# facebookresearch/PartDistillation

Hardware: AMD Instinct MI355X
Metric: images/sec training step, R50 Mask2Former 1024² bs=2/GPU, 1/2/4/8 MI355X (higher is better)
Workload: dtype bf16

## Files before the change

include/pd_gemm.h:

```cpp
#ifndef PD_GEMM_H
#define PD_GEMM_H

#include <stdint.h>

#ifdef __cplusplus
extern "C" {
#endif

int pd_gemm_tn_f32(const float *A, const float *B, const float *bias, float *C, int M, int N, int K, int lda, int ldb,
                   int ldc, int relu, void *stream);

int pd_gemm_tn_f32x3(const float *A, const float *B, const float *bias, float *C, int M, int N, int K, int lda, int ldb,
                     int ldc, int relu, void *stream);

int pd_gemm_wgrad_f32(const float *dY, const float *X, float *dW, float *dB, int M, int N, int K, int ldy, int ldx,
                      int ldw, void *stream);

int pd_gemm_wgrad_acc_f32(const float *dY, const float *X, float *dW, float *dB, int M, int N, int K, int ldy, int ldx,
                          int ldw, void *stream);

int64_t pd_gemm_tn_f32x3_relu_bits_words(int M, int N);
int pd_split3_bf16(const float *W, int N, int K, int ldw, int transpose, void *planes, void *stream);
int pd_gemm_tn_f32x3_pre(const float *A, const void *Bplanes, const float *bias, float *C, uint32_t *bits, float *colsum, int M, int N, int K,
                         int lda, int ldc, int mode, void *stream);
int pd_gemm_tn_f32x3_relu_bits(const float *A, const float *B, const float *bias, float *C, uint32_t *bits, int M, int N, int K, int lda,
                               int ldb, int ldc, void *stream);
int pd_gemm_tn_f32x3_relumask(const float *A, const float *B, const uint32_t *bits, float *C, float *colsum, int M, int N, int K, int lda,
                              int ldb, int ldc, void *stream);

int pd_gemm_wgrad_acc_f32x3(const float *dY, const float *X, float *dW, float *dB, int M, int N, int K, int ldy, int ldx, int ldw,
                            void *stream);
int64_t pd_gemm_wgrad_f32x3_ws_floats(int N, int K);
int pd_gemm_wgrad_acc_f32x3_ws(const float *dY, const float *X, float *dW, float *dB, float *workspace, int64_t workspace_floats, int M, int N,
                               int K, int ldy, int ldx, int ldw, void *stream);

typedef struct PdGemmWgradDesc {
  const float *dY, *X;
  float *dW, *dB;
  int M, N, K, ldy, ldx, ldw;
  const float *y_amax, *x_amax;
} PdGemmWgradDesc;
int64_t pd_gemm_wgrad_f32x3_grouped_table_bytes(int max_count);
int64_t pd_gemm_wgrad_f32x3_grouped_ws_floats(const PdGemmWgradDesc *descs, int count);
int pd_gemm_wgrad_f32x3_grouped(const PdGemmWgradDesc *descs, int count, void *table_host_pinned, void *table_device, float *workspace,
                                int64_t workspace_floats, void *stream);

int pd_conv3x3_wgrad_nhwc_f32x3(const float *dY, const float *X, float *dWk, float *dB, float *workspace, int64_t workspace_floats, int B, int H,
                                int W, int Ci, int Co, void *stream);

int pd_conv3x3_nhwc_f32x3(const float *X, const float *Wk, const float *bias, float *Y, int B, int H, int W, int Ci, int Co,
                          void *stream);

int64_t pd_gemm_wgrad_f16x2_ws_floats(int N, int K);
int pd_gemm_wgrad_f16x2_takes_wide_tiles(int N, int K);
int64_t pd_gemm_wgrad_f16x2_grouped_ws_floats(const PdGemmWgradDesc *descs, int count);
int pd_gemm_wgrad_acc_f16x2_ws(const float *dY, const float *X, float *dW, float *dB, const float *y_amax, const float *x_amax,
                               float *workspace, int64_t workspace_floats, int M, int N, int K, int ldy, int ldx, int ldw, void *stream);
int pd_gemm_wgrad_f16x2_grouped(const PdGemmWgradDesc *descs, int count, void *table_host_pinned, void *table_device, float *workspace,
                                int64_t workspace_floats, void *stream);
int pd_conv3x3_wgrad_nhwc_f16x2(const float *dY, const float *X, float *dWk, float *dB, const float *y_amax, const float *x_amax,
                                float *workspace, int64_t workspace_floats, int B, int H, int W, int Ci, int Co, void *stream);
int pd_gemm_tn_f16x2_which(int M, int N, int K, int mode, int has_bits, int has_amax);

int pd_conv3x3_nhwc_f16x2(const float *X, const float *Wk, const float *bias, float *Y, const float *x_amax, const float *w_amax, float *y_amax,
                          int B, int H, int W, int Ci, int Co, void *stream);
int64_t pd_gemm_tn_f16x2_bits_words(int M, int N);
int pd_gemm_tn_f16x2(const float *A, const float *B, const float *bias, float *C, uint32_t *bits, float *colsum, const float *a_amax,
                     const float *b_amax, float *c_amax, int M, int N, int K, int lda, int ldb, int ldc, int mode, void *stream);
int pd_row_amax_f32(const float *X, int rows, int cols, int ld, float *out, void *stream);
int pd_gemm_tn_f16x2_bf16out(const float *A, const float *B, const float *bias, void *C_bf16, const float *a_amax, const float *b_amax, int M, int N,
                             int K, int lda, int ldb, int ldc, void *stream);
int pd_cast_bf16_f32_amax(const void *X_bf16, int rows, int cols, float *Y, float *row_amax, void *stream);

#ifdef __cplusplus
}
#endif
#endif
```

partdistillation_amd/csrc/common.hip:

```cpp
#include <hip/hip_runtime.h>
#include <stdarg.h>
#include <stdio.h>
#include <string.h>

#include "pd_common.h"
#include "pd_msda.h"

namespace {
thread_local char g_err[512] = {0};
}

int pd_set_error(int code, const char *fmt, ...)
{
  va_list ap;
  va_start(ap, fmt);
  vsnprintf(g_err, sizeof(g_err), fmt, ap);
  va_end(ap);
  return code;
}

int pd_check_launch(const char *what)
{
  hipError_t e = hipGetLastError();
  if (e == hipSuccess) return PD_OK;
  return pd_set_error(PD_ERR_LAUNCH, "%s: %s", what, hipGetErrorString(e));
}

extern "C" const char *pd_last_error(void) { return g_err; }
extern "C" int pd_abi_version(void) { return 39; }

extern int g_pd_dbg_atomic_scope;
extern int g_pd_dbg_force_generic;
extern int g_pd_dbg_ablate;
extern int g_pd_dbg_x3_narrow;
extern int g_pd_dbg_f16x2;
extern int g_pd_dbg_wgrad_wide;
extern "C" void pd_dbg_set_wgrad_xcd(int v);
extern "C" void pd_dbg_set_wgrad_fast(int v);
extern int g_pd_dbg_bwd_variant;
extern int g_pd_dbg_msda_gate_pct;
extern int g_pd_dbg_wgrad_wgs;
extern int g_pd_dbg_bwd_threads;
extern int g_pd_dbg_attn_scalar;
extern int g_pd_dbg_wattn;
extern int g_pd_dbg_x3;
extern int g_pd_dbg_kmeans;
extern int g_pd_dbg_conv_group_rows;
extern int g_pd_dbg_conv_xcd_major;
extern int g_pd_dbg_sgemm_deep;
extern int g_ig_bn, g_ig_nst, g_ig_splits, g_ig_patch, g_ig_pcls;
extern int g_mx_bn, g_mx_nst;
extern int g_swin_ln_abl;
extern int g_ln_bwd_cap;
extern int g_crit_abl;
extern int g_attn_bwd_kc;
extern int g_wg_nst, g_wg_splits, g_wg_mode;
extern "C" int pd_debug_set(const char *key, int value)
{
  if (!key) return PD_ERR_INVALID_ARG;
  if (!strcmp(key, "msda_bwd_atomic_scope")) { g_pd_dbg_atomic_scope = value; return PD_OK; }
  if (!strcmp(key, "msda_ablate")) { g_pd_dbg_ablate = value; return PD_OK; }
  if (!strcmp(key, "msda_bwd_variant")) { g_pd_dbg_bwd_variant = value; return PD_OK; }
  if (!strcmp(key, "msda_gate_pct")) { g_pd_dbg_msda_gate_pct = value; return PD_OK; }
  if (!strcmp(key, "attn_scalar")) { g_pd_dbg_attn_scalar = value; return PD_OK; }
  if (!strcmp(key, "msda_bwd_threads")) { g_pd_dbg_bwd_threads = value; return PD_OK; }
  if (!strcmp(key, "wgrad_wgs")) { g_pd_dbg_wgrad_wgs = value; return PD_OK; }
  if (!strcmp(key, "kmeans_ablate")) { g_pd_dbg_kmeans = value; return PD_OK; }
  if (!strcmp(key, "wg_nst")) { g_wg_nst = value; return PD_OK; }
  if (!strcmp(key, "wg_splits")) { g_wg_splits = value; return PD_OK; }
  if (!strcmp(key, "wg_mode")) { g_wg_mode = value; return PD_OK; }
  if (!strcmp(key, "ig_bn")) { g_ig_bn = value; return PD_OK; }
  if (!strcmp(key, "ig_patch")) { g_ig_patch = value; return PD_OK; }
  if (!strcmp(key, "ig_pcls")) { g_ig_pcls = value; return PD_OK; }
  if (!strcmp(key, "ig_nst")) { g_ig_nst = value; return PD_OK; }
  if (!strcmp(key, "mx_bn")) { g_mx_bn = value; return PD_OK; }
  if (!strcmp(key, "attn_bwd_kc")) { g_attn_bwd_kc = value; return PD_OK; }
  if (!strcmp(key, "crit_abl")) { g_crit_abl = value; return PD_OK; }
  if (!strcmp(key, "ln_bwd_cap")) { g_ln_bwd_cap = value; return PD_OK; }
  if (!strcmp(key, "swin_ln_abl")) { g_swin_ln_abl = value; return PD_OK; }
  if (!strcmp(key, "mx_nst")) { g_mx_nst = value; return PD_OK; }
  if (!strcmp(key, "ig_splits")) { g_ig_splits = value; return PD_OK; }
  if (!strcmp(key, "sgemm_deep")) { g_pd_dbg_sgemm_deep = value; return PD_OK; }
  if (!strcmp(key, "conv_group_rows")) { g_pd_dbg_conv_group_rows = value; return PD_OK; }
  if (!strcmp(key, "conv_xcd_major")) { g_pd_dbg_conv_xcd_major = value; return PD_OK; }
  if (!strcmp(key, "x3_ablate")) { g_pd_dbg_x3 = value; return PD_OK; }
  if (!strcmp(key, "f16x2_tile")) { g_pd_dbg_f16x2 = value; return PD_OK; }
  if (!strcmp(key, "wgrad_wide")) { g_pd_dbg_wgrad_wide = value; return PD_OK; }
  if (!strcmp(key, "wgrad_xcd")) { pd_dbg_set_wgrad_xcd(value); return PD_OK; }
  if (!strcmp(key, "wgrad_fast")) { pd_dbg_set_wgrad_fast(value); return PD_OK; }
  if (!strcmp(key, "x3_narrow")) { g_pd_dbg_x3_narrow = value; return PD_OK; }
  if (!strcmp(key, "wattn_ablate")) { g_pd_dbg_wattn = value; return PD_OK; }
  if (!strcmp(key, "msda_force_generic")) { g_pd_dbg_force_generic = value; return PD_OK; }
  return pd_set_error(PD_ERR_INVALID_ARG, "pd_debug_set: unknown key %s", key);
}
```

partdistillation_amd/csrc/gemm_f16x2.hip:

```cpp
#include <hip/hip_runtime.h>
#include <stdint.h>
#include <stdlib.h>
#include <type_traits>

#include "f16x2.h"
#include "pd_common.h"
#include "xcd.h"
#include "pd_gemm.h"
#include "pd_msda.h"

#ifndef PD_ABL
#define PD_ABL 0
#endif

namespace {
using namespace pdh2;
__device__ __forceinline__ int xcd_chunk(int bid, int nb) { return pd_xcd_chunk(bid, nb); }
__device__ __forceinline__ unsigned short f2bf_rne(float f)
{
  unsigned u = __float_as_uint(f);
  if ((u & 0x7fffffffu) > 0x7f800000u) return (unsigned short)((u >> 16) | 0x40u);
  u += 0x7fffu + ((u >> 16) & 1u);
  return (unsigned short)(u >> 16);
}
// ... 1023 lines not shown
      static bool battr = false;
      if (!battr) {
        (void)hipFuncSetAttribute((const void *)(gemm_kpc_f16x2<true, 0, true>), hipFuncAttributeMaxDynamicSharedMemorySize, (int)KP_LDS);
        (void)hipFuncSetAttribute((const void *)(gemm_kpc_f16x2<false, 0, true>), hipFuncAttributeMaxDynamicSharedMemorySize, (int)KP_LDS);
        (void)hipFuncSetAttribute((const void *)(gemm_kpc_f16x2<true, 16, true>), hipFuncAttributeMaxDynamicSharedMemorySize, (int)KP_LDS);
        battr = true;
      }
      const float *bpl = reinterpret_cast<const float *>(planes);
      if (dbg == 234) hipLaunchKernelGGL((gemm_kpc_f16x2<true, 16, true>), dim3((unsigned)G), dim3(768), KP_LDS, st, A, bpl, bias, C, M, K, lda, ldb, ldc, np, a_amax, b_amax, 0, 0);
      else if (a_amax) hipLaunchKernelGGL((gemm_kpc_f16x2<true, 0, true>), dim3((unsigned)G), dim3(768), KP_LDS, st, A, bpl, bias, C, M, K, lda, ldb, ldc, np, a_amax, b_amax, 0, 0);
      else hipLaunchKernelGGL((gemm_kpc_f16x2<false, 0, true>), dim3((unsigned)G), dim3(768), KP_LDS, st, A, bpl, bias, C, M, K, lda, ldb, ldc, np, a_amax, b_amax, 0, 0);
      return pd_check_launch("pd_gemm_tn_f16x2 (producer / consumer wavefronts, weight planes)");
    }
#endif
    if (a_amax) hipLaunchKernelGGL(gemm_kpc_f16x2<true>, dim3((unsigned)G), dim3(768), KP_LDS, st, A, B, bias, C, M, K, lda, ldb, ldc, np, a_amax, b_amax, 0, 0);
    else hipLaunchKernelGGL(gemm_kpc_f16x2<false>, dim3((unsigned)G), dim3(768), KP_LDS, st, A, B, bias, C, M, K, lda, ldb, ldc, np, a_amax, b_amax, 0, 0);
    return pd_check_launch("pd_gemm_tn_f16x2 (producer / consumer wavefronts)");
  }
  const bool need_wide = bits != nullptr;
  if (need_wide && ((N % 256) || M < 1024)) return pd_set_error(PD_ERR_INVALID_ARG, "pd_gemm_tn_f16x2: sign bits need N %% 256 == 0 and M >= 1024");
  const bool wide_ok = (N % 256) == 0 && M >= 1024;
  const bool by_shape = dbg == 0 || dbg == 61 || dbg == 70 || dbg == 80 || dbg == 62;
  static const bool wide_deepk = []() { const char *e = getenv("PD_H2_WIDE_DEEPK"); return e && e[0] == '1'; }();
  const bool wide = need_wide || dbg == 3 || dbg == 13 || (by_shape && wide_ok && (int64_t)((M + 255) / 256) * (N / 256) >= 128 && (N >= 1024 || (K >= 512 && wide_deepk)));
  static const bool fast_env = []() { const char *e = getenv("PD_H2_FAST"); return !e || e[0] != '0'; }();
#define GO(TM, TN, WN, NRS, FAST) return launch_f16x2<TM, TN, WN, 16, false, NRS, FAST>(A, B, bias, C, M, N, K, lda, ldb, ldc, mode, bits, colsum, a_amax, b_amax, c_amax, st, flags)
  if (wide) {
    if (!wide_ok) return pd_set_error(PD_ERR_INVALID_ARG, "pd_gemm_tn_f16x2: 256 x 256 tiles need N %% 256 == 0 and M >= 1024");
    if (dbg == 3) GO(256, 256, 128, 1, 0);
    if (dbg == 13 || dbg == 70) GO(256, 256, 128, 2, 0);
    if (!fast_env) GO(256, 256, 128, 2, 0);
    GO(256, 256, 128, 2, 1);
  }
  if (dbg == 4 || dbg == 70) GO(128, 128, 64, 1, 0);
  if (dbg == 14 || !fast_env) GO(128, 128, 64, 2, 0);
  GO(128, 128, 64, 2, 1);
#undef GO
}

extern "C" int pd_gemm_tn_f16x2_which(int M, int N, int K, int mode, int has_bits, int has_amax)
{
  const int dbg = g_pd_dbg_f16x2;
  static const bool rows_k256 = []() { const char *e = getenv("PD_H2_ROWS_K256"); return !e || e[0] != '0'; }();
  if ((dbg == 61 || (rows_k256 && dbg == 0)) && mode == 0 && K == 256 && (N % 256) == 0 && M >= 8192) return 2;
#ifdef PD_PROBES
  if ((dbg == 90 || (dbg >= 100 && dbg < 132)) && mode == 0 && K == 256 && M >= 4096 && (N % 32) == 0 && N >= 96 && ((N % 128) == 0 || (N % 96) == 0)) return 3;
#endif
  if (dbg != 62 && dbg != 3 && dbg != 13 && dbg != 70 && (mode == 1 || mode == 2) && has_bits && K == 256 && (N % 256) == 0 && N >= 512 && M >= 8192 && has_amax && g_rows_relu) return 2;
  static const bool kpc_env = []() { const char *e = getenv("PD_H2_KPC"); return !e || e[0] != '0'; }();
  if (((kpc_env && dbg == 0) || dbg == 92 || dbg == 93) && mode == 0 && !has_bits && K >= 512 && (K % KR_KC) == 0 && (N % 256) == 0 && N <= 512 && M >= 8192 && kpc_items_ok(M, N)) return 5;
#ifdef PD_PROBES
  static const bool kres_env = []() { const char *e = getenv("PD_H2_KRES"); return e && e[0] == '1'; }();
  if (((kres_env && dbg == 0) || dbg == 91) && mode == 0 && !has_bits && K >= 512 && (K % KR_KC) == 0 && (N % 256) == 0 && N <= 512 && M >= 8192) return 4;
#endif
  const bool wide_ok = (N % 256) == 0 && M >= 1024;
  const bool by_shape = dbg == 0 || dbg == 61 || dbg == 70 || dbg == 80 || dbg == 62;
  static const bool wide_deepk = []() { const char *e = getenv("PD_H2_WIDE_DEEPK"); return e && e[0] == '1'; }();
  const bool wide = has_bits || dbg == 3 || dbg == 13 || (by_shape && wide_ok && (int64_t)((M + 255) / 256) * (N / 256) >= 128 && (N >= 1024 || (K >= 512 && wide_deepk)));
  return wide ? 1 : 0;
}

extern "C" int pd_gemm_tn_f16x2(const float *A, const float *B, const float *bias, float *C, uint32_t *bits, float *colsum, const float *a_amax,
                                const float *b_amax, float *c_amax, int M, int N, int K, int lda, int ldb, int ldc, int mode, void *stream_)
{
  return gemm_tn_f16x2_impl(A, B, bias, C, bits, colsum, a_amax, b_amax, c_amax, M, N, K, lda, ldb, ldc, mode, stream_, 0);
}

extern "C" int pd_gemm_tn_f16x2_bf16out(const float *A, const float *B, const float *bias, void *C_bf16, const float *a_amax, const float *b_amax,
                                        int M, int N, int K, int lda, int ldb, int ldc, void *stream_)
{
  return gemm_tn_f16x2_impl(A, B, bias, reinterpret_cast<float *>(C_bf16), nullptr, nullptr, a_amax, b_amax, nullptr, M, N, K, lda, ldb, ldc, 0, stream_, 1);
}

extern "C" int pd_cast_bf16_f32_amax(const void *X_bf16, int rows, int cols, float *Y, float *row_amax, void *stream_)
{
  if (rows < 0 || cols <= 0 || (cols & 7)) return pd_set_error(PD_ERR_INVALID_ARG, "pd_cast_bf16_f32_amax: rows=%d cols=%d (a multiple of 8)", rows, cols);
  if (rows == 0) return PD_OK;
  if (!X_bf16 || !Y || !row_amax || ((uintptr_t)X_bf16 & 15) || ((uintptr_t)Y & 15)) return pd_set_error(PD_ERR_INVALID_ARG, "pd_cast_bf16_f32_amax: null / misaligned pointer");
  hipLaunchKernelGGL(cast_bf16_f32_amax, dim3((unsigned)((rows + 3) / 4)), dim3(256), 0, (hipStream_t)stream_, (const unsigned short *)X_bf16, rows, cols, Y,
                     row_amax);
  return pd_check_launch("pd_cast_bf16_f32_amax");
}

extern "C" int pd_conv3x3_nhwc_f16x2(const float *X, const float *Wk, const float *bias, float *Y, const float *x_amax, const float *w_amax,
                                     float *y_amax, int B, int H, int W, int Ci, int Co, void *stream_)
{
  if (B < 0 || H <= 0 || W <= 0 || Ci <= 0 || Co <= 0 || (Ci & 15))
    return pd_set_error(PD_ERR_INVALID_ARG, "pd_conv3x3_nhwc_f16x2: B=%d H=%d W=%d Ci=%d (%% 16) Co=%d", B, H, W, Ci, Co);
  if (B == 0) return PD_OK;
  if (!X || !Wk || !Y || ((uintptr_t)X & 15) || ((uintptr_t)Wk & 15)) return pd_set_error(PD_ERR_INVALID_ARG, "pd_conv3x3_nhwc_f16x2: null / misaligned pointer");
  const int64_t M = (int64_t)B * H * W;
  if (M > 0x7fffffffLL - 4096) return pd_set_error(PD_ERR_INVALID_ARG, "pd_conv3x3_nhwc_f16x2: too many pixels");
  hipStream_t st = (hipStream_t)stream_;
#ifdef PD_PROBES
  static const bool kpc_conv = []() { const char *e = getenv("PD_H2_KPC_CONV"); return e && e[0] == '1'; }();
  if (((kpc_conv && g_pd_dbg_f16x2 == 0) || g_pd_dbg_f16x2 == 92 || g_pd_dbg_f16x2 == 234) && x_amax && w_amax && !y_amax && (Co % 256) == 0 && (Ci % KR_KC) == 0 && ((Ci / KR_KC) & (Ci / KR_KC - 1)) == 0 && M >= 8192 &&
      H < 65536 && W < 65536 && M * Ci * 4 < (1ll << 31) && (int64_t)Co * 9 * Ci * 4 < (1ll << 31)) {
    static int ncu5 = 0;
    if (!ncu5) { int dev = 0; (void)hipGetDevice(&dev); if (hipDeviceGetAttribute(&ncu5, hipDeviceAttributeMultiprocessorCount, dev) != hipSuccess || ncu5 < 8) ncu5 = 256; }
    const int np = Co / 256, nwork = (int)((M + KR_RB - 1) / KR_RB) * np, G = nwork < ncu5 ? nwork : ncu5;
    static bool cattr = false;
    if (!cattr) {
      (void)hipFuncSetAttribute((const void *)(gemm_kpc_f16x2<true, 0, false, true>), hipFuncAttributeMaxDynamicSharedMemorySize, (int)KP_LDS);
      cattr = true;
    }
    if (g_pd_dbg_f16x2 == 234) {
      (void)hipFuncSetAttribute((const void *)(gemm_kpc_f16x2<true, 16, false, true>), hipFuncAttributeMaxDynamicSharedMemorySize, (int)KP_LDS);
      hipLaunchKernelGGL((gemm_kpc_f16x2<true, 16, false, true>), dim3((unsigned)G), dim3(768), KP_LDS, st, X, Wk, bias, Y, (int)M, 9 * Ci, Ci, 9 * Ci, Co, np, x_amax,
                         w_amax, H, W);
      return pd_check_launch("pd_conv3x3_nhwc_f16x2 (producer / consumer wavefronts, stamps)");
    }
    hipLaunchKernelGGL((gemm_kpc_f16x2<true, 0, false, true>), dim3((unsigned)G), dim3(768), KP_LDS, st, X, Wk, bias, Y, (int)M, 9 * Ci, Ci, 9 * Ci, Co, np, x_amax,
                       w_amax, H, W);
    return pd_check_launch("pd_conv3x3_nhwc_f16x2 (producer / consumer wavefronts)");
  }
#endif
  const bool wide = g_pd_dbg_f16x2 == 3 || (g_pd_dbg_f16x2 != 4 && (Co % 256) == 0 && M >= 65536);
  if (g_pd_dbg_f16x2 == 70 || g_pd_dbg_f16x2 == 21) {
    if (wide) return launch_f16x2<256, 256, 128, 16, true>(X, Wk, bias, Y, (int)M, Co, 9 * Ci, Ci, 9 * Ci, Co, 0, nullptr, nullptr, x_amax, w_amax, y_amax, st, H, W);
    return launch_f16x2<128, 128, 64, 16, true>(X, Wk, bias, Y, (int)M, Co, 9 * Ci, Ci, 9 * Ci, Co, 0, nullptr, nullptr, x_amax, w_amax, y_amax, st, H, W);
  }
  if (wide) return launch_f16x2<256, 256, 128, 16, true, 1, 1>(X, Wk, bias, Y, (int)M, Co, 9 * Ci, Ci, 9 * Ci, Co, 0, nullptr, nullptr, x_amax, w_amax, y_amax, st, H, W);
  return launch_f16x2<128, 128, 64, 16, true, 1, 1>(X, Wk, bias, Y, (int)M, Co, 9 * Ci, Ci, 9 * Ci, Co, 0, nullptr, nullptr, x_amax, w_amax, y_amax, st, H, W);
}

extern "C" int pd_row_amax_f32(const float *X, int rows, int cols, int ld, float *out, void *stream_)
{
  if (rows < 0 || cols < 0) return pd_set_error(PD_ERR_INVALID_ARG, "pd_row_amax_f32: negative size");
  if (rows == 0) return PD_OK;
  if (!X || !out) return pd_set_error(PD_ERR_INVALID_ARG, "pd_row_amax_f32: null pointer");
  hipLaunchKernelGGL(row_amax_f32, dim3((unsigned)((rows + 3) / 4)), dim3(256), 0, (hipStream_t)stream_, X, rows, cols, ld, out);
  return pd_check_launch("pd_row_amax_f32");
}

extern "C" int pd_debug_read_kpc_trace(unsigned long long *dst)
{
  return hipMemcpyFromSymbol(dst, HIP_SYMBOL(g_kp_trace), sizeof(unsigned long long) * 2 * 64 * 8) == hipSuccess ? PD_OK : PD_ERR_LAUNCH;
}
```

partdistillation_amd/lib.py:

```python
import ctypes
import os
import subprocess

_HERE = os.path.dirname(os.path.abspath(__file__))
LIB_PATH = os.environ.get("PD_LIB_PATH") or os.path.join(_HERE, "libpd_hip.so")
CSRC = os.path.join(_HERE, "csrc")

PD_F32, PD_F64, PD_BF16 = 0, 1, 2
ABI_VERSION = 39

_c_int, _c_vp = ctypes.c_int, ctypes.c_void_p

SIGNATURES = {
    "pd_msda_forward": (_c_int, [_c_vp] * 6 + [_c_int] * 9 + [_c_vp]),
    "pd_msda_backward": (_c_int, [_c_vp] * 9 + [_c_int] * 9 + [_c_vp]),
    "pd_msda_backward_last_gate": (_c_int, [_c_vp]),
    "pd_stem7x7_fwd": (_c_int, [_c_vp, _c_int] + [_c_vp] * 4 + [_c_int] * 4 + [_c_vp]),
    "pd_stem_wgrad_workspace_floats": (ctypes.c_int64, []),
    "pd_stem7x7_wgrad": (_c_int, [_c_vp, _c_int] + [_c_vp] * 4 + [_c_int, _c_vp] + [_c_int] * 4 + [_c_vp]),
    "pd_msda_fused_supported": (_c_int, [_c_int] * 7),
    "pd_msda_fused_forward": (_c_int, [_c_vp] * 4 + [_c_int] + [_c_vp] * 4 + [_c_int] * 7 + [_c_vp]),
    "pd_msda_fused_backward": (_c_int, [_c_vp] * 4 + [_c_int] + [_c_vp] * 6 + [_c_int, _c_vp, _c_vp] + [_c_int] * 7 + [_c_vp]),
    "pd_lsa_batched": (_c_int, [_c_vp] * 4 + [_c_int] * 3 + [_c_vp]),
    "pd_sumsq_accumulate": (_c_int, [_c_vp, ctypes.c_int64, _c_int, _c_vp, _c_vp]),
    "pd_adamw_clipped": (_c_int, [_c_vp] * 4 + [ctypes.c_int64, _c_int] + [ctypes.c_double] * 5 + [_c_int, _c_vp, ctypes.c_double, _c_vp, _c_vp]),
    "pd_gemm_tn_f32": (_c_int, [_c_vp] * 4 + [_c_int] * 7 + [_c_vp]),
    "pd_gemm_tn_f32x3": (_c_int, [_c_vp] * 4 + [_c_int] * 7 + [_c_vp]),
    "pd_gemm_wgrad_f16x2_takes_wide_tiles": (_c_int, [_c_int] * 2),
    "pd_gemm_wgrad_f16x2_ws_floats": (ctypes.c_int64, [_c_int] * 2),
    "pd_gemm_wgrad_f16x2_grouped_ws_floats": (ctypes.c_int64, [_c_vp, _c_int]),
    "pd_gemm_wgrad_acc_f16x2_ws": (_c_int, [_c_vp] * 7 + [ctypes.c_int64] + [_c_int] * 6 + [_c_vp]),
    "pd_gemm_wgrad_f16x2_grouped": (_c_int, [_c_vp, _c_int, _c_vp, _c_vp, _c_vp, ctypes.c_int64, _c_vp]),
    "pd_conv3x3_wgrad_nhwc_f16x2": (_c_int, [_c_vp] * 7 + [ctypes.c_int64] + [_c_int] * 5 + [_c_vp]),
    "pd_conv3x3_nhwc_f16x2": (_c_int, [_c_vp] * 7 + [_c_int] * 5 + [_c_vp]),
    "pd_gemm_tn_f16x2_which": (_c_int, [_c_int] * 6),
    "pd_gemm_tn_f16x2_bits_words": (ctypes.c_int64, [_c_int] * 2),
    "pd_gemm_tn_f16x2": (_c_int, [_c_vp] * 9 + [_c_int] * 7 + [_c_vp]),
    "pd_gemm_tn_f16x2_bf16out": (_c_int, [_c_vp] * 6 + [_c_int] * 6 + [_c_vp]),
    "pd_cast_bf16_f32_amax": (_c_int, [_c_vp, _c_int, _c_int, _c_vp, _c_vp, _c_vp]),
    "pd_row_amax_f32": (_c_int, [_c_vp, _c_int, _c_int, _c_int, _c_vp, _c_vp]),
    "pd_gemm_tn_f32x3_relumask": (_c_int, [_c_vp] * 5 + [_c_int] * 6 + [_c_vp]),
    "pd_gemm_tn_f32x3_relu_bits": (_c_int, [_c_vp] * 5 + [_c_int] * 6 + [_c_vp]),
    "pd_gemm_tn_f32x3_relu_bits_words": (ctypes.c_int64, [_c_int] * 2),
    "pd_split3_bf16": (_c_int, [_c_vp, _c_int, _c_int, _c_int, _c_int, _c_vp, _c_vp]),
    "pd_gemm_tn_f32x3_pre": (_c_int, [_c_vp] * 6 + [_c_int] * 6 + [_c_vp]),
    "pd_gemm_wgrad_f32": (_c_int, [_c_vp] * 4 + [_c_int] * 6 + [_c_vp]),
    "pd_gemm_wgrad_acc_f32": (_c_int, [_c_vp] * 4 + [_c_int] * 6 + [_c_vp]),
    "pd_conv3x3_nhwc_f32x3": (_c_int, [_c_vp] * 4 + [_c_int] * 5 + [_c_vp]),
    "pd_gemm_wgrad_acc_f32x3": (_c_int, [_c_vp] * 4 + [_c_int] * 6 + [_c_vp]),
    "pd_conv3x3_wgrad_nhwc_f32x3": (_c_int, [_c_vp] * 5 + [ctypes.c_int64] + [_c_int] * 5 + [_c_vp]),
    "pd_gemm_wgrad_f32x3_ws_floats": (ctypes.c_int64, [_c_int] * 2),
    "pd_gemm_wgrad_f32x3_grouped_table_bytes": (ctypes.c_int64, [_c_int]),
    "pd_gemm_wgrad_f32x3_grouped_ws_floats": (ctypes.c_int64, [_c_vp, _c_int]),
    "pd_gemm_wgrad_f32x3_grouped": (_c_int, [_c_vp, _c_int, _c_vp, _c_vp, _c_vp, ctypes.c_int64, _c_vp]),
    "pd_gemm_wgrad_acc_f32x3_ws": (_c_int, [_c_vp] * 5 + [ctypes.c_int64] + [_c_int] * 6 + [_c_vp]),
    "pd_adamw_clipped_shadow": (_c_int, [_c_vp] * 5 + [ctypes.c_int64] + [ctypes.c_double] * 5 + [_c_int, _c_vp, ctypes.c_double, _c_vp, _c_vp]),
    "pd_conv_bf16_supported": (_c_int, [_c_int] * 5),
    "pd_conv_bf16_fwd": (_c_int, [_c_vp] * 6 + [_c_int] * 11 + [_c_vp]),
    "pd_conv_bf16_wgrad_workspace_floats": (ctypes.c_int64, [_c_int] * 6),
    "pd_conv_bf16_wgrad": (_c_int, [_c_vp] * 4 + [ctypes.c_int64] + [_c_int] * 10 + [_c_vp]),
    "pd_conv_bf16_wgrad_grouped_table_bytes": (ctypes.c_int64, [_c_int]),
    "pd_conv_bf16_wgrad_grouped_workspace_floats": (ctypes.c_int64, [_c_vp, _c_int]),
    "pd_conv_bf16_wgrad_grouped": (_c_int, [_c_vp, _c_int, _c_vp, _c_vp, _c_vp, ctypes.c_int64, _c_vp]),
    "pd_conv_bf16_dgrad": (_c_int, [_c_vp] * 4 + [_c_int] * 10 + [_c_vp]),
    "pd_maxpool3s2_fwd_bf16": (_c_int, [_c_vp] * 3 + [_c_int] * 4 + [_c_vp]),
    "pd_maxpool3s2_bwd_bf16": (_c_int, [_c_vp] * 3 + [_c_int] * 4 + [_c_vp]),
    "pd_affine_act_fwd_bf16": (_c_int, [_c_vp] * 5 + [ctypes.c_int64, _c_int, _c_int, _c_vp]),
    "pd_affine_act_bwd_bf16": (_c_int, [_c_vp] * 5 + [ctypes.c_int64, _c_int, _c_int, _c_vp]),
    "pd_affine_act_bwd2_bf16": (_c_int, [_c_vp] * 6 + [ctypes.c_int64, _c_int, _c_int, _c_vp]),
    "pd_multi_gather_sumsq": (_c_int, [_c_vp] * 8 + [_c_int, _c_int, _c_vp]),
    "pd_attn_workspace_floats": (ctypes.c_int64, [_c_int] * 4),
    "pd_attn_fwd_d32": (_c_int, [_c_vp] * 7 + [_c_int] * 4 + [ctypes.c_float, _c_int, _c_vp]),
    "pd_attn_bwd_d32": (_c_int, [_c_vp] * 11 + [_c_int] * 4 + [ctypes.c_float, _c_int, _c_vp]),
    "pd_attn_fwd_d32_ld": (_c_int, [_c_vp] * 7 + [_c_int] * 4 + [ctypes.c_float, _c_int, _c_int, _c_vp]),
    "pd_attn_bwd_d32_ld": (_c_int, [_c_vp] * 11 + [_c_int] * 4 + [ctypes.c_float, _c_int, _c_int, _c_vp]),
    "pd_nc_sums_f32": (_c_int, [_c_vp] * 6 + [_c_int] * 5 + [_c_vp]),
    "pd_nc_affine_f32": (_c_int, [_c_vp] * 4 + [_c_int] * 4 + [_c_vp]),
    "pd_nc_affine_amax_f32": (_c_int, [_c_vp] * 5 + [_c_int] * 4 + [_c_vp]),
    "pd_nc_affine2_amax_f32": (_c_int, [_c_vp] * 8 + [_c_int] * 4 + [_c_vp]),
    "pd_upsample_add_amax_nhwc_f32": (_c_int, [_c_vp, ctypes.c_int64] + [_c_vp] * 3 + [_c_int] * 6 + [_c_vp]),
    "pd_nc_affine2_f32": (_c_int, [_c_vp] * 7 + [_c_int] * 4 + [_c_vp]),
    "pd_add_layernorm_fwd": (_c_int, [_c_vp, _c_int, _c_vp, _c_vp, _c_vp, ctypes.c_float, _c_vp, _c_vp, _c_vp, _c_vp, _c_int, _c_vp,
                                      _c_int, _c_vp, _c_vp, _c_int, _c_int, _c_vp]),
    "pd_add_layernorm_bwd": (_c_int, [_c_vp] * 4 + [_c_int] + [_c_vp] * 6 + [_c_int] + [_c_vp] * 4 + [_c_int] * 3 + [_c_vp]),
    "pd_add_layernorm_fwd_amax": (_c_int, [_c_vp, _c_int, _c_vp, _c_vp, _c_vp, ctypes.c_float, _c_vp, _c_vp, _c_vp, _c_vp, _c_int, _c_vp,
                                           _c_int, _c_vp, _c_vp, _c_vp, _c_vp, _c_int, _c_int, _c_vp]),
    "pd_add_layernorm_bwd_amax": (_c_int, [_c_vp] * 4 + [_c_int] + [_c_vp] * 6 + [_c_int] + [_c_vp] * 4 + [_c_int] + [_c_vp] + [_c_int] * 2 + [_c_vp]),
    "pd_colsum_acc": (_c_int, [_c_vp, _c_int, _c_int, _c_int, _c_vp, _c_vp]),
    "pd_relu_bwd_colsum": (_c_int, [_c_vp, _c_vp, _c_int, _c_int, _c_int, _c_vp, _c_vp]),
    "pd_mem_prep_fwd": (_c_int, [_c_vp, ctypes.c_int64, _c_vp, _c_vp, _c_vp, _c_vp, _c_int, _c_int, _c_int, _c_int, _c_vp]),
    "pd_mem_prep_bwd": (_c_int, [_c_vp, _c_vp, _c_int, _c_vp, ctypes.c_int64, _c_int, _c_int, _c_int, _c_vp]),
    "pd_attn_mask_u8": (_c_int, [_c_vp, _c_int, _c_int, _c_int, _c_vp, _c_vp]),
    "pd_add_rows_amax_f32": (_c_int, [_c_vp] * 6 + [_c_int, _c_int, _c_vp]),
    "pd_sum3_sum2_f32": (_c_int, [_c_vp] * 6 + [ctypes.c_int64, _c_vp]),
    "pd_transpose_batched_f32": (_c_int, [_c_vp, _c_int, _c_vp]),
    "pd_normalize_u8_nhwc": (_c_int, [_c_vp, _c_int, _c_int, _c_int, _c_vp, _c_vp, _c_vp, _c_vp]),
    "pd_resize_bilinear_nhwc_f32": (_c_int, [_c_vp] + [_c_int] * 4 + [_c_vp] * 3 + [_c_int, _c_int, _c_vp]),
    "pd_matcher_point_terms": (_c_int, [_c_vp, _c_int, _c_int, _c_int, _c_vp, _c_vp, _c_vp, _c_vp, _c_vp]),
    "pd_match_point_logits": (_c_int, [_c_vp] * 4 + [_c_int] * 7 + [_c_vp]),
    "pd_matcher_costs": (_c_int, [_c_vp, _c_int, _c_vp] + [ctypes.c_int64] * 3 + [_c_vp] * 3 + [_c_int] * 6 + [ctypes.c_float] * 3 + [_c_vp]),
    "pd_mask_point_losses_fwd": (_c_int, [_c_vp] * 5 + [_c_int, _c_int, _c_vp]),
    "pd_mask_point_losses_bwd": (_c_int, [_c_vp] * 6 + [_c_int, _c_int, _c_vp]),
    "pd_uncertain_points": (_c_int, [_c_vp] * 4 + [_c_int] * 4 + [_c_vp]),
    "pd_point_sample_u8": (_c_int, [_c_vp] * 4 + [_c_int] * 5 + [_c_vp]),
    "pd_skinny_linear_fwd": (_c_int, [_c_vp] * 3 + [_c_int, _c_vp] + [_c_int] * 3 + [_c_vp]),
    "pd_skinny_linear_partial_floats": (ctypes.c_int64, [_c_int] * 3),
    "pd_skinny_linear_bwd": (_c_int, [_c_vp, _c_vp, _c_int, _c_vp, _c_vp, _c_vp, _c_int, _c_vp, _c_vp, _c_vp] + [_c_int] * 4 + [_c_vp]),
    "pd_loss_vectors_fwd": (_c_int, [_c_vp, ctypes.c_int64, ctypes.c_int64] + [_c_vp] * 9 + [_c_int] * 5 + [_c_vp]),
    "pd_loss_vectors_bwd": (_c_int, [_c_vp, ctypes.c_int64, ctypes.c_int64] + [_c_vp] * 10 + [_c_int] * 5 + [_c_vp]),
    "pd_pair_logits_fwd": (_c_int, [_c_vp] * 5 + [_c_int] * 4 + [_c_vp]),
    "pd_pair_logits_bwd_tok": (_c_int, [_c_vp] * 5 + [_c_int] * 4 + [_c_vp]),
    "pd_pair_logits_workspace_floats": (ctypes.c_int64, [_c_int] * 3),
    "pd_pair_logits_bwd_rows": (_c_int, [_c_vp] * 6 + [_c_int] * 4 + [_c_vp]),
    "pd_msda_prep_fwd": (_c_int, [_c_vp] * 6 + [ctypes.c_int64] + [_c_int] * 5 + [_c_vp]),
    "pd_msda_prep_bwd_amax": (_c_int, [_c_vp] * 7 + [ctypes.c_int64] + [_c_int] * 5 + [_c_vp]),
    "pd_msda_forward_amax": (_c_int, [_c_vp] * 7 + [_c_int] * 9 + [_c_vp]),
    "pd_msda_prep_bwd": (_c_int, [_c_vp] * 6 + [ctypes.c_int64] + [_c_int] * 5 + [_c_vp]),
    "pd_sgemm_tn_batched_bf16": (_c_int, [_c_vp] * 3 + [_c_int] * 7 + [ctypes.c_int64] * 3 + [_c_vp]),
# ... 150 lines not shown
```

Baseline: 107.4.

## Add patch-based implicit-GEMM 3x3 conv kernel with pre-split f16x2 weight planes

Adds a new forward 3x3 NHWC conv path that stages an input halo patch (tile plus one-pixel border) in LDS once per channel chunk and reuses it across all nine taps. The previous path was an im2col-style implicit GEMM with K=9*Ci. Weights are pre-split into hi/lo f16 planes by a separate kernel on every call, and weight loads are double-buffered against the MFMA compute. The aim is to cut redundant global and LDS traffic for the input. In exchange it adds an extra weight-split launch per call and a lazily allocated per-device workspace, and it falls back when the stream is being captured.

Measured after the change: 108.4, median of 6. About the same (+0.9%).

```diff
diff --git a/include/pd_gemm.h b/include/pd_gemm.h
--- a/include/pd_gemm.h
+++ b/include/pd_gemm.h
@@ -64,6 +64,7 @@
 
 int pd_conv3x3_nhwc_f16x2(const float *X, const float *Wk, const float *bias, float *Y, const float *x_amax, const float *w_amax, float *y_amax,
                           int B, int H, int W, int Ci, int Co, void *stream);
+int pd_conv3x3_nhwc_f16x2_which(int B, int H, int W, int Ci, int Co, int has_amax);
 int64_t pd_gemm_tn_f16x2_bits_words(int M, int N);
 int pd_gemm_tn_f16x2(const float *A, const float *B, const float *bias, float *C, uint32_t *bits, float *colsum, const float *a_amax,
                      const float *b_amax, float *c_amax, int M, int N, int K, int lda, int ldb, int ldc, int mode, void *stream);
diff --git a/partdistillation_amd/csrc/common.hip b/partdistillation_amd/csrc/common.hip
--- a/partdistillation_amd/csrc/common.hip
+++ b/partdistillation_amd/csrc/common.hip
@@ -34,6 +34,7 @@
 extern int g_pd_dbg_ablate;
 extern int g_pd_dbg_x3_narrow;
 extern int g_pd_dbg_f16x2;
+extern int g_h2_conv_patch;
 extern int g_pd_dbg_wgrad_wide;
 extern "C" void pd_dbg_set_wgrad_xcd(int v);
 extern "C" void pd_dbg_set_wgrad_fast(int v);
@@ -85,6 +86,7 @@
   if (!strcmp(key, "conv_xcd_major")) { g_pd_dbg_conv_xcd_major = value; return PD_OK; }
   if (!strcmp(key, "x3_ablate")) { g_pd_dbg_x3 = value; return PD_OK; }
   if (!strcmp(key, "f16x2_tile")) { g_pd_dbg_f16x2 = value; return PD_OK; }
+  if (!strcmp(key, "h2_conv_patch")) { g_h2_conv_patch = value; return PD_OK; }
   if (!strcmp(key, "wgrad_wide")) { g_pd_dbg_wgrad_wide = value; return PD_OK; }
   if (!strcmp(key, "wgrad_xcd")) { pd_dbg_set_wgrad_xcd(value); return PD_OK; }
   if (!strcmp(key, "wgrad_fast")) { pd_dbg_set_wgrad_fast(value); return PD_OK; }
diff --git a/partdistillation_amd/csrc/conv3x3_patch_f16x2.hip b/partdistillation_amd/csrc/conv3x3_patch_f16x2.hip
--- /dev/null
+++ b/partdistillation_amd/csrc/conv3x3_patch_f16x2.hip
@@ -0,0 +1,250 @@
+#include <hip/hip_runtime.h>
+#include <stdint.h>
+#include <stdlib.h>
+
+#include "f16x2.h"
+#include "pd_common.h"
+#include "xcd.h"
+#include "pd_gemm.h"
+#include "pd_msda.h"
+
+namespace {
+using namespace pdh2;
+typedef unsigned cp_u32x4 __attribute__((ext_vector_type(4)));
+
+constexpr int CP_TW = 16, CP_PW = CP_TW + 2;
+constexpr int CP_CC = 32;
+constexpr int CP_BT = 2 * 2 * 256 * 16;
+template <int TH> struct CpGeo {
+  static constexpr int NW = TH / 2, NTH = NW * 64, PIX = (TH + 2) * CP_PW;
+  static constexpr int PAN = PIX * 16;
+  static constexpr int PATCH = 2 * (CP_CC / 8) * PAN;
+  static constexpr int ITEMS = PIX * (CP_CC / 4);
+  static constexpr int NLD = (ITEMS + NTH - 1) / NTH;
+  static constexpr int NB = (CP_BT / 16) / NTH;
+  static constexpr size_t LDS = (size_t)2 * PATCH + 2 * CP_BT + 2 * 256 * sizeof(float) + NW * sizeof(float);
+};
+
+__device__ __forceinline__ int cp_perm(int r) { return r < 4 ? r : r < 12 ? r + 12 : r < 16 ? r - 8 : r < 20 ? r + 8 : r < 28 ? r - 12 : r; }
+
+__global__ __launch_bounds__(256) void conv3x3_split_w_f16x2(const float *__restrict__ Wk, const float *__restrict__ w_amax, uint4 *__restrict__ Wp,
+                                                             int Ci, int Co)
+{
+  const int g8n = Ci >> 3;
+  const int idx = blockIdx.x * 256 + threadIdx.x;
+  if (idx >= Co * 9 * g8n) return;
+  const int g = idx % g8n, rest = idx / g8n, tap = rest % 9, co = rest / 9;
+  const float4 *src = reinterpret_cast<const float4 *>(Wk + ((int64_t)co * 9 + tap) * Ci + g * 8);
+  float s, inv;
+  row_scale(w_amax[co], s, inv);
+  const SplitH a = split4h_u(src[0], s), b = split4h_u(src[1], s);
+  const int nb = co >> 8, n = co & 255, c = g >> 2, ks = (g >> 1) & 1, pan = g & 1;
+  uint4 *d = Wp + ((((int64_t)nb * (Ci / CP_CC) + c) * 9 + tap) * 2 + ks) * (CP_BT / 16) + pan * 256 + n;
+  d[0] = make_uint4(a.hi.x, a.hi.y, b.hi.x, b.hi.y);
+  d[512] = make_uint4(a.lo.x, a.lo.y, b.lo.x, b.lo.y);
+}
+
+template <int TH>
+__global__ __launch_bounds__(TH * 32, 16 / TH) void conv3x3_patch_f16x2(const float *__restrict__ X, const uint4 *__restrict__ Wp, const float *__restrict__ bias,
+                                                                        float *__restrict__ Y, const float *__restrict__ x_amax, const float *__restrict__ w_amax,
+                                                                        int H, int W, int Ci, int Co, int txn, int tyn, int ncb)
+{
+  typedef CpGeo<TH> G;
+  constexpr int NTH = G::NTH, PAN = G::PAN, WR = TH / 4;
+  extern __shared__ __attribute__((aligned(16))) unsigned char smem[];
+  unsigned char *const patch = smem;
+  unsigned char *const bst = smem + 2 * G::PATCH;
+  float *const s_iw = reinterpret_cast<float *>(bst + 2 * CP_BT);
+  float *const s_bias = s_iw + 256;
+  float *const s_red = s_bias + 256;
+  const int t = threadIdx.x, lane = t & 63, wave = t >> 6;
+  const int lb = pd_xcd_chunk(blockIdx.x, gridDim.x);
+  const int nb = lb % ncb, mt = lb / ncb;
+  const int b = mt / (tyn * txn), r_ = mt - b * (tyn * txn), ty0 = (r_ / txn) * TH, tx0 = (r_ - (r_ / txn) * txn) * CP_TW;
+  const int n0 = nb * 256;
+
+  float pm = 0.f;
+  for (int i = t; i < G::PIX; i += NTH) {
+    const int py = i / CP_PW, px = i - py * CP_PW, sy = ty0 - 1 + py, sx = tx0 - 1 + px;
+    if ((unsigned)sy < (unsigned)H && (unsigned)sx < (unsigned)W) pm = fmaxf(pm, x_amax[((int64_t)b * H + sy) * W + sx]);
+  }
+#pragma unroll
+  for (int o = 32; o; o >>= 1) pm = fmaxf(pm, __shfl_xor(pm, o, 64));
+  if (lane == 0) s_red[wave] = pm;
+  for (int i = t; i < 256; i += NTH) {
+    float s, inv;
+    row_scale(w_amax[n0 + i], s, inv);
+    s_iw[i] = inv;
+    s_bias[i] = bias ? bias[n0 + i] : 0.f;
+  }
+  __syncthreads();
+  pm = s_red[0];
+#pragma unroll
+  for (int w = 1; w < G::NW; ++w) pm = fmaxf(pm, s_red[w]);
+  float xs, xinv;
+  row_scale(pm, xs, xinv);
+
+  int poff[G::NLD];
+  unsigned pok = 0;
+#pragma unroll
+  for (int j = 0; j < G::NLD; ++j) {
+    const int item = t + NTH * j, pix = item >> 3, q = item & 7;
+    const int py = pix / CP_PW, px = pix - py * CP_PW, sy = ty0 - 1 + py, sx = tx0 - 1 + px;
+    const bool in = item < G::ITEMS && (unsigned)sy < (unsigned)H && (unsigned)sx < (unsigned)W;
+    const int cy = min(max(sy, 0), H - 1), cx = min(max(sx, 0), W - 1);
+    poff[j] = ((b * H + cy) * W + cx) * Ci + q * 4;
+    pok |= (in ? 1u : 0u) << j;
+  }
+  const int pdst = ((t & 7) >> 1) * PAN + (t >> 3) * 16 + (t & 1) * 8;
+  float4 ra[G::NLD];
+  auto pload = [&](int c) __attribute__((always_inline)) {
+#pragma unroll
+    for (int j = 0; j < G::NLD; ++j) ra[j] = *reinterpret_cast<const float4 *>(X + poff[j] + c * CP_CC);
+  };
+  auto pstore = [&](int buf) __attribute__((always_inline)) {
+#pragma unroll
+    for (int j = 0; j < G::NLD; ++j) {
+      if (j < G::NLD - 1 || t + NTH * j < G::ITEMS) {
+        const bool in = (pok >> j) & 1u;
+        const float4 v = make_float4(in ? ra[j].x : 0.f, in ? ra[j].y : 0.f, in ? ra[j].z : 0.f, in ? ra[j].w : 0.f);
+        const SplitH x = split4h_u(v, xs);
+        unsigned char *p = patch + buf * G::PATCH + pdst + 2 * NTH * j;
+        *reinterpret_cast<uint2 *>(p) = x.hi;
+        *reinterpret_cast<uint2 *>(p + (CP_CC / 8) * PAN) = x.lo;
+      }
+    }
+  };
+  const int nch = Ci / CP_CC, S = nch * 18;
+  const cp_u32x4 *wsrc = reinterpret_cast<const cp_u32x4 *>(Wp) + (int64_t)nb * S * (CP_BT / 16) + t;
+  cp_u32x4 rb[G::NB];
+  auto bload = [&](int s) __attribute__((always_inline)) {
+#pragma unroll
+    for (int u = 0; u < G::NB; ++u) rb[u] = wsrc[s * (CP_BT / 16) + NTH * u];
+  };
+  auto bstore = [&](int buf) __attribute__((always_inline)) {
+#pragma unroll
+    for (int u = 0; u < G::NB; ++u) *reinterpret_cast<cp_u32x4 *>(bst + buf * CP_BT + (t + NTH * u) * 16) = rb[u];
+  };
+
+  f32x16 acc[4][2];
+#pragma unroll
+  for (int j = 0; j < 4; ++j)
+#pragma unroll
+    for (int i = 0; i < 2; ++i)
+#pragma unroll
+      for (int e = 0; e < 16; ++e) acc[j][i][e] = 0.f;
+  const int fr = lane & 31, fh = lane >> 5, wr = wave % WR, wc = wave / WR;
+  const int qp = cp_perm(fr);
+  int pb[2];
+#pragma unroll
+  for (int i = 0; i < 2; ++i) pb[i] = ((4 * wr + 2 * i + (qp >> 4)) * CP_PW + (qp & 15)) * 16 + fh * PAN;
+  const int bb = (wc * 128 + fr) * 16 + fh * 4096;
+  auto compute = [&](const unsigned char *P, const unsigned char *Bs) __attribute__((always_inline)) {
+    h16x8 a[2][2], w[2][4];
+#pragma unroll
+    for (int pl = 0; pl < 2; ++pl) {
+#pragma unroll
+      for (int j = 0; j < 4; ++j) w[pl][j] = *reinterpret_cast<const h16x8 *>(Bs + pl * 8192 + bb + j * 512);
+#pragma unroll
+      for (int i = 0; i < 2; ++i) a[pl][i] = *reinterpret_cast<const h16x8 *>(P + pl * 4 * PAN + pb[i]);
+    }
+#define PTERM(PW, PA)                                                        \
+  _Pragma("unroll") for (int j = 0; j < 4; ++j)                              \
+      _Pragma("unroll") for (int i = 0; i < 2; ++i) mmah(acc[j][i], w[PW][j], a[PA][i]);
+    PTERM(1, 0)
+    PTERM(0, 1)
+    PTERM(0, 0)
+#undef PTERM
+  };
+
+  pload(0);
+  bload(0);
+  pstore(0);
+  bstore(0);
+  bload(1);
+  __syncthreads();
+  for (int c = 0; c < nch; ++c) {
+    const unsigned char *P = patch + (c & 1) * G::PATCH;
+    const bool more = c + 1 < nch;
+#pragma unroll
+    for (int tap = 0; tap < 9; ++tap)
+#pragma unroll
+      for (int ks = 0; ks < 2; ++ks) {
+        const int s = (c * 9 + tap) * 2 + ks;
+        if (s + 1 < S) bstore(ks ^ 1);
+        if (s + 2 < S) bload(s + 2);
+        if (ks == 0 && tap == 0 && more) pload(c + 1);
+        if (ks == 0 && tap == 4 && more) pstore((c + 1) & 1);
+        compute(P + 2 * ks * PAN + ((tap / 3) * CP_PW + tap % 3) * 16, bst + ks * CP_BT);
+        __syncthreads();
+      }
+  }
+
+#pragma unroll
+  for (int i = 0; i < 2; ++i) {
+    const int y = ty0 + 4 * wr + 2 * i + (qp >> 4), x = tx0 + (qp & 15);
+    if (y >= H || x >= W) continue;
+    float *yp = Y + (((int64_t)b * H + y) * W + x) * Co + n0 + wc * 128 + 4 * fh;
+#pragma unroll
+    for (int j = 0; j < 4; ++j)
+#pragma unroll
+      for (int g = 0; g < 4; ++g) {
+        const int cl = wc * 128 + j * 32 + 8 * g + 4 * fh;
+        const float4 iw = *reinterpret_cast<const float4 *>(s_iw + cl), bv = *reinterpret_cast<const float4 *>(s_bias + cl);
+        *reinterpret_cast<float4 *>(yp + j * 32 + 8 * g) =
+            make_float4(acc[j][i][4 * g] * (xinv * iw.x) + bv.x, acc[j][i][4 * g + 1] * (xinv * iw.y) + bv.y,
+                        acc[j][i][4 * g + 2] * (xinv * iw.z) + bv.z, acc[j][i][4 * g + 3] * (xinv * iw.w) + bv.w);
+      }
+  }
+}
+}
+
+int g_h2_conv_patch = []() { const char *e = getenv("PD_H2_CONV_PATCH"); return e ? atoi(e) : 1; }();
+
+bool conv3x3_patch_f16x2_applies(int B, int H, int W, int Ci, int Co, bool has_amax, bool has_y_amax)
+{
+  const int64_t M = (int64_t)B * H * W;
+  return g_h2_conv_patch != 0 && has_amax && !has_y_amax && B > 0 && (Ci % CP_CC) == 0 && (Co % 256) == 0 && M * Ci * 4 < (1ll << 31) &&
+         M * Co * 4 < (1ll << 31) && (int64_t)Co * 9 * Ci * 4 < (1ll << 31);
+}
+
+int conv3x3_patch_f16x2_launch(const float *X, const float *Wk, const float *bias, float *Y, const float *x_amax, const float *w_amax, int B, int H,
+                               int W, int Ci, int Co, hipStream_t st)
+{
+  static uint4 *planes[16] = {nullptr};
+  static int64_t planes_cap[16] = {0};
+  int dev = 0;
+  (void)hipGetDevice(&dev);
+  if (dev < 0 || dev >= 16) return 1;
+  const int64_t need = (int64_t)Co * 9 * Ci * 4;
+  if (need > planes_cap[dev]) {
+    hipStreamCaptureStatus cs = hipStreamCaptureStatusNone;
+    (void)hipStreamIsCapturing(st, &cs);
+    if (cs != hipStreamCaptureStatusNone) return 1;
+    if (planes[dev]) (void)hipFree(planes[dev]);
+    planes[dev] = nullptr;
+    planes_cap[dev] = 0;
+    if (hipMalloc(reinterpret_cast<void **>(&planes[dev]), (size_t)need) != hipSuccess) {
+      (void)hipGetLastError();
+      planes[dev] = nullptr;
+      return pd_set_error(PD_ERR_LAUNCH, "pd_conv3x3_nhwc_f16x2: no memory for the weight planes");
+    }
+    planes_cap[dev] = need;
+  }
+  const int nw = Co * 9 * (Ci / 8);
+  hipLaunchKernelGGL(conv3x3_split_w_f16x2, dim3((unsigned)((nw + 255) / 256)), dim3(256), 0, st, Wk, w_amax, planes[dev], Ci, Co);
+  const int th = g_h2_conv_patch == 8 ? 8 : 16;
+  const int txn = (W + CP_TW - 1) / CP_TW, tyn = (H + th - 1) / th, ncb = Co / 256;
+  const dim3 grid((unsigned)((int64_t)B * tyn * txn * ncb));
+  static bool attr = false;
+  if (!attr) {
+    (void)hipFuncSetAttribute((const void *)conv3x3_patch_f16x2<8>, hipFuncAttributeMaxDynamicSharedMemorySize, (int)CpGeo<8>::LDS);
+    (void)hipFuncSetAttribute((const void *)conv3x3_patch_f16x2<16>, hipFuncAttributeMaxDynamicSharedMemorySize, (int)CpGeo<16>::LDS);
+    attr = true;
+  }
+  if (th == 16)
+    hipLaunchKernelGGL(conv3x3_patch_f16x2<16>, grid, dim3(CpGeo<16>::NTH), CpGeo<16>::LDS, st, X, planes[dev], bias, Y, x_amax, w_amax, H, W, Ci, Co, txn, tyn, ncb);
+  else
+    hipLaunchKernelGGL(conv3x3_patch_f16x2<8>, grid, dim3(CpGeo<8>::NTH), CpGeo<8>::LDS, st, X, planes[dev], bias, Y, x_amax, w_amax, H, W, Ci, Co, txn, tyn, ncb);
+  return pd_check_launch("pd_conv3x3_nhwc_f16x2 (patch form)");
+}
diff --git a/partdistillation_amd/csrc/gemm_f16x2.hip b/partdistillation_amd/csrc/gemm_f16x2.hip
--- a/partdistillation_amd/csrc/gemm_f16x2.hip
+++ b/partdistillation_amd/csrc/gemm_f16x2.hip
@@ -1129,6 +1129,10 @@
   return pd_check_launch("pd_cast_bf16_f32_amax");
 }
 
+bool conv3x3_patch_f16x2_applies(int B, int H, int W, int Ci, int Co, bool has_amax, bool has_y_amax);
+int conv3x3_patch_f16x2_launch(const float *X, const float *Wk, const float *bias, float *Y, const float *x_amax, const float *w_amax, int B, int H,
+                               int W, int Ci, int Co, hipStream_t st);
+
 extern "C" int pd_conv3x3_nhwc_f16x2(const float *X, const float *Wk, const float *bias, float *Y, const float *x_amax, const float *w_amax,
                                      float *y_amax, int B, int H, int W, int Ci, int Co, void *stream_)
 {
@@ -1139,6 +1143,10 @@
   const int64_t M = (int64_t)B * H * W;
   if (M > 0x7fffffffLL - 4096) return pd_set_error(PD_ERR_INVALID_ARG, "pd_conv3x3_nhwc_f16x2: too many pixels");
   hipStream_t st = (hipStream_t)stream_;
+  if (g_pd_dbg_f16x2 == 0 && conv3x3_patch_f16x2_applies(B, H, W, Ci, Co, x_amax && w_amax, y_amax != nullptr) && !((uintptr_t)Y & 15)) {
+    const int rc = conv3x3_patch_f16x2_launch(X, Wk, bias, Y, x_amax, w_amax, B, H, W, Ci, Co, st);
+    if (rc != 1) return rc;
+  }
 #ifdef PD_PROBES
   static const bool kpc_conv = []() { const char *e = getenv("PD_H2_KPC_CONV"); return e && e[0] == '1'; }();
   if (((kpc_conv && g_pd_dbg_f16x2 == 0) || g_pd_dbg_f16x2 == 92 || g_pd_dbg_f16x2 == 234) && x_amax && w_amax && !y_amax && (Co % 256) == 0 && (Ci % KR_KC) == 0 && ((Ci / KR_KC) & (Ci / KR_KC - 1)) == 0 && M >= 8192 &&
@@ -1171,6 +1179,12 @@
   return launch_f16x2<128, 128, 64, 16, true, 1, 1>(X, Wk, bias, Y, (int)M, Co, 9 * Ci, Ci, 9 * Ci, Co, 0, nullptr, nullptr, x_amax, w_amax, y_amax, st, H, W);
 }
 
+extern "C" int pd_conv3x3_nhwc_f16x2_which(int B, int H, int W, int Ci, int Co, int has_amax)
+{
+  if (g_pd_dbg_f16x2 == 0 && conv3x3_patch_f16x2_applies(B, H, W, Ci, Co, has_amax != 0, false)) return 2;
+  return (g_pd_dbg_f16x2 == 3 || (g_pd_dbg_f16x2 != 4 && (Co % 256) == 0 && (int64_t)B * H * W >= 65536)) ? 1 : 0;
+}
+
 extern "C" int pd_row_amax_f32(const float *X, int rows, int cols, int ld, float *out, void *stream_)
 {
   if (rows < 0 || cols < 0) return pd_set_error(PD_ERR_INVALID_ARG, "pd_row_amax_f32: negative size");
diff --git a/partdistillation_amd/lib.py b/partdistillation_amd/lib.py
--- a/partdistillation_amd/lib.py
+++ b/partdistillation_amd/lib.py
@@ -34,6 +34,7 @@
     "pd_conv3x3_wgrad_nhwc_f16x2": (_c_int, [_c_vp] * 7 + [ctypes.c_int64] + [_c_int] * 5 + [_c_vp]),
     "pd_conv3x3_nhwc_f16x2": (_c_int, [_c_vp] * 7 + [_c_int] * 5 + [_c_vp]),
     "pd_gemm_tn_f16x2_which": (_c_int, [_c_int] * 6),
+    "pd_conv3x3_nhwc_f16x2_which": (_c_int, [_c_int] * 6),
     "pd_gemm_tn_f16x2_bits_words": (ctypes.c_int64, [_c_int] * 2),
     "pd_gemm_tn_f16x2": (_c_int, [_c_vp] * 9 + [_c_int] * 7 + [_c_vp]),
     "pd_gemm_tn_f16x2_bf16out": (_c_int, [_c_vp] * 6 + [_c_int] * 6 + [_c_vp]),
```
